# getzlab/rnaseqc

Measured on AMD Instinct MI355X. Metric: reads/sec whole-node (100 M-read synthetic BAM, GENCODE GTF) at 1/2/4/8 GPU -- `value`: the hot path over the records resident in HBM (the bench contract's definition of value); `whole_node.value`: the same job from the BAM file to the reports (CLI `Average Reads/Sec` window), checked against `value, higher is better.
Workload: dtype i32/u64 counters, f64 exon fractions

## Files before the change

rnaseqc_amd/csrc/rsqc_device.h:

```cpp
#pragma once

#if !defined(RSQC_WAVE_EMU)
#include <hip/hip_runtime.h>
#endif
#include <stdint.h>

#include "rsqc_read.h"

#define RSQC_K1_THREADS 256
#define RSQC_MAX_BIAS_WINDOW 1024
#define RSQC_K3_THREADS 1024
#include "rsqc_k3_plan.h"

namespace rsqc {

struct DevBatch {
    uint64_t n;
    uint64_t record_base;
    const rsqc_rec_core *core;
    const rsqc_rec_aux *aux;
    const uint32_t *cigar;
    const uint32_t *qhash2;
    uint32_t n_seg;
    const int32_t *seg_tid;
    const uint64_t *seg_start;
    const uint64_t *seg_file_index;
    uint32_t n_wide;
    const uint64_t *wide_index;
    const int32_t *wide_nm, *wide_l_qseq;
    const uint32_t *wide_n_cigar;
};

RSQC_HD uint64_t batch_file_index(const DevBatch &b, uint32_t seg, uint64_t i) {
    return b.seg_file_index ? b.seg_file_index[seg] + (i - b.seg_start[seg]) : b.record_base + i;
}

struct FragCandidates {
    uint64_t *file_index;
    uint64_t *qhash;
    int32_t *name;
    int32_t *endpos;
    uint32_t *flag_size;
    uint32_t *count; uint32_t cap;
    uint32_t *chunk_count;
    uint32_t *h2;
};

struct DevReference {
    const unsigned long long *bits;
    const unsigned long long *word_off;
    const unsigned long long *length;
};
struct GcCandidates {
    uint64_t *file_index;
    uint64_t *qhash;
    uint32_t *row;
    int32_t *endpos;
    uint32_t *flag_lq;
    int32_t *tid;
    uint32_t *count; uint32_t cap;
    uint32_t *h2;
};
__device__ __forceinline__ uint32_t gc_count(const DevReference &R, int contig, int64_t s, int64_t e) {
    if (e <= s) return 0u;
    const unsigned long long *w = R.bits + R.word_off[contig];
    const int64_t w0 = s >> 6, w1 = (e - 1) >> 6;
    uint32_t n = 0;
    for (int64_t i = w0; i <= w1; ++i) {
        unsigned long long x = w[i];
        if (i == w0) x &= ~0ull << (s & 63);
        if (i == w1) x &= ~0ull >> (63 - ((e - 1) & 63));
        n += (uint32_t)__popcll(x);
    }
    return n;
}
__device__ __forceinline__ double gc_value(uint32_t k, uint64_t size) {
    const double inc = 1.0 / (double)size;
    double c = 0.0;
    for (uint32_t i = 0; i < k; ++i) c += inc;
    return c;
}

struct alignas(16) PairRec { uint32_t gene, h2; uint64_t hash; };
struct DevAccum {
    unsigned long long *gene_reads, *gene_unique, *gene_frag, *counters;
    double *exon_acc;
    uint32_t *cov_diff;
    PairRec *pairs;
    uint32_t pair_chunk_cap; uint32_t *pair_chunk_count;
    uint32_t pair_slow_base, pair_slow_cap; uint32_t *pair_slow_count;
    uint32_t *ovf_count; uint64_t *ovf_index; uint32_t ovf_cap;
    uint32_t *defer_index; uint32_t *defer_list; uint32_t *defer_total;
    uint32_t *tile_span;
    FragCandidates frag;
    uint32_t *rl_stats;
    uint32_t *rl_seg;
    int32_t *read_length;
    int *error;
};

struct GeneCovArgs {
    const uint32_t *ge_off, *ge_row;
    const ExonRow *ex;
    const uint32_t *ex_cov;
    const uint32_t *ex_id;
    const uint32_t *gene_cov_off;
    const uint32_t *gene_coding;
    const uint8_t *gene_flags;
    const uint8_t *gene_owned;
    const uint32_t *gene_order;
    const unsigned long long *gene_reads;
    uint32_t *cov;
    int32_t n_listed;
    uint32_t mask; int32_t bias_offset, bias_window; uint64_t bias_gene_length;
    double *g_mean, *g_std, *g_cv; uint8_t *g_valid;
    double *e_cv; uint8_t *e_cv_valid;
    unsigned long long *bias3, *bias5;
    int *error;
};
void launch_gene_coverage(hipStream_t s, hipStream_t s2, hipStream_t s3, const GeneCovArgs &A, uint32_t n_large, uint32_t n_medium, uint32_t n_xlarge,
                          uint32_t n_le6144 = 0, uint32_t n_le3072 = 0, uint32_t n_le2048 = 0, uint32_t n_le1024 = 0);

void launch_reduce_add(hipStream_t s, unsigned long long *du, const unsigned long long *su, size_t nu, double *df, const double *sf, size_t nf,
                       uint8_t *db, const uint8_t *sb, size_t nb);
void launch_pack_results(hipStream_t s, const double *exon_acc, uint8_t *exon_hit, uint32_t n_exons);
void launch_reset(hipStream_t s, void *arena, size_t arena_bytes, void *cov, size_t cov_bytes, uint32_t *rl_min);
void launch_classify(hipStream_t s, int grid, int variant, const DevAnnotation &a, const DevParams &p, const DevBatch &b,
                     const DevAccum &acc);
inline int rsqc_long_grid(int k1_grid) { return k1_grid < 1024 ? k1_grid : 1024; }
void launch_classify_long(hipStream_t s, int k1_grid, const DevAnnotation &a, const DevParams &p, const DevBatch &b, const DevAccum &acc);
void launch_ei_rank(hipStream_t s, const EiEntry *ei, uint32_t ei_lo, uint32_t ei_hi, EiRank *rank, uint32_t n_words);
void launch_classify_slow(hipStream_t s, const DevAnnotation &a, const DevParams &p, const DevBatch &b,
                          const DevAccum &acc);
#define RSQC_RL_SUMMARY_WORDS (2 + 2 * 128)
void launch_read_length(hipStream_t s, const DevAnnotation &a, const DevParams &p, const DevBatch &b,
                        const DevAccum &acc, uint32_t *summary);
#define RSQC_SLOW_RES 2048u
#define RSQC_SLOW_LEGACY_GRID 4096u
#ifndef RSQC_K4_PART_READS
#define RSQC_K4_PART_READS 1024
#endif
#define RSQC_K4_SUB_CAP (2 * RSQC_K4_PART_READS)
#define RSQC_K4_PART_SLOTS (4 * RSQC_K4_PART_READS)
#ifndef RSQC_K4_COUNT_THREADS
#define RSQC_K4_COUNT_THREADS 256
#endif
struct FragKey { uint32_t lo, hi, h2; };
struct FragPlan {
    uint32_t *part_first;
    uint32_t *cursor;
    uint4 *ginfo;
    uint4 *part_info;
    uint32_t *full_list, *full_n;
    FragKey *list;
    unsigned long long *blk_space; uint32_t *blk_parts;
};
void launch_frag_layout(hipStream_t s, const unsigned long long *gene_reads, uint32_t n_genes, const FragPlan &P, int *error);
void launch_frag_local(hipStream_t s, const DevAccum &acc, uint32_t n_chunks, const FragPlan &P, uint32_t list_blocks);
void launch_pairs_append(hipStream_t s, const PairRec *src, uint32_t chunk_cap, const uint32_t *counts,
                         uint32_t n_chunks, uint32_t slow_base, uint32_t slow_cap, PairRec *dst);
void launch_frag_count(hipStream_t s, uint32_t n_genes, const FragPlan &P, uint32_t parts_bound, unsigned long long *gene_frag, int *error);

}

#include <vector>
namespace rsqc {
struct SortScratch { void *k0 = nullptr, *k1 = nullptr, *v0 = nullptr, *v1 = nullptr, *v2 = nullptr, *v3 = nullptr, *tmp = nullptr, *count = nullptr;
                     size_t cap_n = 0, tmp_bytes = 0; uint32_t *table = nullptr, *out_size = nullptr, *out_count = nullptr; };
void free_sort_scratch(SortScratch &s);
int run_fragment_sizes(hipStream_t stream, const FragCandidates &c, uint32_t n, uint32_t max_samples,
                       std::vector<int64_t> &sizes, std::vector<uint64_t> &counts, uint32_t &remaining, SortScratch &S, uint32_t &n_kept, int *d_error);
void launch_frag_compact(hipStream_t s, const FragCandidates &src, const FragCandidates &dst, uint64_t n_rec, int k1_grid);
void launch_gc_pack(hipStream_t s, const uint8_t *ascii, uint64_t len, unsigned long long *words);
void launch_exon_gc(hipStream_t s, const DevAnnotation &a, const DevReference &R, double *exon_gc);
void launch_gc_candidates(hipStream_t s, const DevAnnotation &a, const DevParams &p, const DevBatch &b, const DevReference &R,
                          const GcCandidates &out, int *error);
int run_gc_content(hipStream_t stream, const GcCandidates &c, uint32_t n, const DevReference &R, unsigned long long *bins, SortScratch &scratch, int *d_error);
}
```

rnaseqc_amd/csrc/rsqc_k4.h:

```cpp
#pragma once

namespace rsqc {


__device__ __forceinline__ uint32_t frag_part_hash(uint64_t key) {
    uint32_t h = (uint32_t)(key >> 32);
    h ^= h >> 15; h *= 0x2C1B3C6Du; h ^= h >> 12;
    return h;
}
__device__ __forceinline__ uint32_t frag_parts_of(unsigned long long reads) {
    return (uint32_t)((reads + RSQC_K4_PART_READS - 1) / RSQC_K4_PART_READS);
}
__device__ __forceinline__ uint32_t frag_cap_of(unsigned long long reads) {
    return frag_parts_of(reads) == 1 ? (uint32_t)reads : (uint32_t)RSQC_K4_SUB_CAP;
}
__device__ __forceinline__ unsigned long long frag_space_of(unsigned long long reads) {
    return ((unsigned long long)frag_parts_of(reads) * frag_cap_of(reads) + 15ull) & ~15ull;
}
__global__ void __launch_bounds__(1024)
frag_layout_totals_kernel(const unsigned long long *gene_reads, uint32_t n_genes, unsigned long long *blk_space, uint32_t *blk_parts, int *error) {
    __shared__ unsigned long long w_space[16];
    __shared__ uint32_t w_parts[16];
    const uint32_t g = blockIdx.x * 1024u + threadIdx.x;
    unsigned long long space = 0; uint32_t parts = 0;
// ... 65 lines not shown
constexpr int k4l_log2(unsigned v) { return v <= 1 ? 0 : 1 + k4l_log2(v >> 1); }
#ifndef RSQC_K4L_WIN
#define RSQC_K4L_WIN 2048
#endif
#ifndef RSQC_K4L_CHUNKS
#define RSQC_K4L_CHUNKS 2
#endif
inline uint32_t frag_local_chunk_wgs(uint32_t n_chunks) { return (n_chunks + RSQC_K4L_CHUNKS - 1u) / RSQC_K4L_CHUNKS; }
struct K4LocalShared {
    uint32_t gkey[RSQC_K4L_GSLOTS], gcnt[RSQC_K4L_GSLOTS];
    unsigned long long win[RSQC_K4L_WIN];
    uint32_t win2[RSQC_K4L_WIN];
};

#ifdef __HIPCC__
#ifndef RSQC_K4L_WAVES
#define RSQC_K4L_WAVES 6
#endif
#define RSQC_K4L_OCC __attribute__((amdgpu_waves_per_eu(RSQC_K4L_WAVES, RSQC_K4L_WAVES)))
#else
#define RSQC_K4L_OCC
#endif
__global__ void __launch_bounds__(RSQC_K4L_THREADS) RSQC_K4L_OCC
frag_local_kernel(const PairRec *pairs, uint32_t chunk_cap,
                  const uint32_t *chunk_count, uint32_t n_chunks, uint32_t slow_base, uint32_t slow_cap,
                  const uint4 *ginfo, uint32_t *cursor, FragKey *list, int *error) {
    __shared__ K4LocalShared S;
    constexpr int CH = RSQC_K4L_CHUNKS;
    const uint32_t n_cwg = (n_chunks + (uint32_t)CH - 1u) / (uint32_t)CH;
    uint32_t cbase[CH], cend[CH];
    uint32_t count, piece0 = 0; constexpr uint32_t piece_step = 1;
    if (blockIdx.x < n_cwg) {
        uint32_t run = 0;
#pragma unroll
        for (int k = 0; k < CH; ++k) {
            const uint32_t c = blockIdx.x * (uint32_t)CH + (uint32_t)k;
            const uint32_t n = c < n_chunks ? (chunk_count[c] < chunk_cap ? chunk_count[c] : chunk_cap) : 0u;
            cbase[k] = c * chunk_cap; run += n; cend[k] = run;
        }
        count = run;
    } else {
#pragma unroll
        for (int k = 0; k < CH; ++k) { cbase[k] = slow_base; cend[k] = 0u; }
        count = chunk_count[n_chunks] < slow_cap ? chunk_count[n_chunks] : slow_cap;
        cend[CH - 1] = count;
#pragma unroll
        for (int k = 0; k < CH - 1; ++k) cend[k] = 0u;
    }
    if (count == 0u) return;
    constexpr int U = RSQC_K4L_PIECE / RSQC_K4L_THREADS;
    constexpr uint32_t NONE = 0xFFFFFFFFu;
    uint32_t n_pieces = (count + RSQC_K4L_PIECE - 1) / RSQC_K4L_PIECE;
    if (blockIdx.x >= n_cwg) {
        const uint32_t sharers = gridDim.x - n_cwg, me = blockIdx.x - n_cwg;
        const uint32_t per = (n_pieces + sharers - 1) / sharers;
        piece0 = me * per < n_pieces ? me * per : n_pieces;
        n_pieces = piece0 + per < n_pieces ? piece0 + per : n_pieces;
    }
    auto pair_at = [&](uint32_t j) -> uint32_t {
        uint32_t at = cbase[CH - 1] + (j - (CH > 1 ? cend[CH - 2] : 0u));
#pragma unroll
        for (int k = CH - 2; k >= 0; --k) if (j < cend[k]) at = cbase[k] + (j - (k > 0 ? cend[k - 1] : 0u));
        return at;
    };
    auto load_piece = [&](uint32_t piece, uint32_t (&g)[U], uint64_t (&key)[U], uint32_t (&h2)[U]) {
#pragma unroll
        for (int u = 0; u < U; ++u) {
            const uint32_t j = piece * RSQC_K4L_PIECE + (uint32_t)u * RSQC_K4L_THREADS + threadIdx.x;
            const bool ok = piece < n_pieces && j < count;
            PairRec r{NONE, 0u, 0ull};
            if (ok) r = pairs[pair_at(j)];
            g[u] = r.gene; key[u] = r.hash; h2[u] = r.h2;
        }
    };
#ifdef RSQC_K1_PROF
    if (blockIdx.x == 1000 && n_chunks > 1000) {
        for (uint32_t i = threadIdx.x; i < count && i < 32768u; i += blockDim.x) { g_dbg_pair_hash[i] = pairs[pair_at(i)].hash; g_dbg_pair_gene[i] = pairs[pair_at(i)].gene; }
        if (threadIdx.x == 0) g_dbg_pair_count = count;
    }
#endif
    uint32_t g[U]; uint64_t key[U]; uint32_t h2[U];
    load_piece(piece0, g, key, h2);
    for (int i = threadIdx.x; i < RSQC_K4L_WIN; i += blockDim.x) { S.win[i] = 0ull; S.win2[i] = 0u; }
    RSQC_FIN_BEGIN
    for (uint32_t piece = piece0; piece < n_pieces; piece += piece_step) {
        RSQC_FIN_SECT(32, 0);
        uint4 gi[U];
#pragma unroll
        for (int u = 0; u < U; ++u) { const uint32_t gq = g[u] != NONE ? g[u] : 0u; gi[u] = ginfo[gq]; }
        uint32_t gn[U]; uint64_t keyn[U]; uint32_t h2n[U];
        load_piece(piece + piece_step, gn, keyn, h2n);
        __syncthreads();
        for (int i = threadIdx.x; i < RSQC_K4L_GSLOTS; i += blockDim.x) { S.gkey[i] = NONE; S.gcnt[i] = 0u; }
        __syncthreads();
        RSQC_FIN_SECT(32, 1);
        uint32_t gp[U], gslot[U], rank[U];
#pragma unroll
        for (int u = 0; u < U; ++u) {
            gslot[u] = NONE; rank[u] = 0; gp[u] = 0;
            if (key[u] == 0) key[u] = 0x9e3779b97f4a7c15ull;
            if (g[u] == NONE) continue;
            {
                unsigned long long lk = key[u] ^ (((unsigned long long)g[u] << 32) | (unsigned long long)(g[u] * 0x9E3779B1u));
                if (lk == 0ull) lk = 1ull;
                static_assert((RSQC_K4L_WIN & (RSQC_K4L_WIN - 1)) == 0, "window size");
                const uint32_t ws = ((((uint32_t)lk ^ (uint32_t)(lk >> 32)) * 0x9E3779B1u) >> 12) & (RSQC_K4L_WIN - 1);
                const bool seen1 = atomicExch(&S.win[ws], lk) == lk, seen2 = atomicExch(&S.win2[ws], h2[u]) == h2[u];
                if (seen1 && seen2) { g[u] = NONE; continue; }
            }
            gp[u] = gi[u].x + (gi[u].y > 1 ? (uint32_t)(((unsigned long long)frag_part_hash(key[u]) * gi[u].y) >> 32) : 0u);
            static_assert((RSQC_K4L_GSLOTS & (RSQC_K4L_GSLOTS - 1)) == 0, "slot hash");
            uint32_t sl = (gp[u] * 0x9E3779B1u) >> (32 - k4l_log2(RSQC_K4L_GSLOTS));
#pragma unroll 1
            for (int probe = 0; probe < 16; ++probe) {
                const uint32_t o = atomicCAS(&S.gkey[sl], NONE, gp[u]);
                if (o == NONE || o == gp[u]) { gslot[u] = sl; rank[u] = atomicAdd(&S.gcnt[sl], 1u); break; }
                sl = (sl + 1) & (RSQC_K4L_GSLOTS - 1);
            }
        }
        RSQC_FIN_SECT(32, 3);
        __syncthreads();
        RSQC_FIN_SECT(32, 4);
        {
            constexpr int R = RSQC_K4L_GSLOTS / RSQC_K4L_THREADS;
            uint32_t pk[R], pc[R], pr[R];
#pragma unroll
            for (int j = 0; j < R; ++j) { pk[j] = S.gkey[j * RSQC_K4L_THREADS + threadIdx.x]; pc[j] = S.gcnt[j * RSQC_K4L_THREADS + threadIdx.x]; }
#pragma unroll
            for (int j = 0; j < R; ++j) pr[j] = pk[j] != NONE ? atomicAdd(&cursor[pk[j]], pc[j]) : 0u;
#pragma unroll
            for (int j = 0; j < R; ++j) S.gcnt[j * RSQC_K4L_THREADS + threadIdx.x] = pr[j];
        }
        __syncthreads();
        RSQC_FIN_SECT(32, 5);
#pragma unroll
        for (int u = 0; u < U; ++u) {
            if (g[u] == NONE) continue;
            const uint32_t at = gslot[u] != NONE ? S.gcnt[gslot[u]] + rank[u] : atomicAdd(&cursor[gp[u]], 1u);
            const uint32_t cap = gi[u].z;
            if (at < cap) {
                const unsigned long long where = ((unsigned long long)gi[u].w << 4) + (unsigned long long)(gp[u] - gi[u].x) * cap + at;
                list[where] = FragKey{(uint32_t)key[u], (uint32_t)(key[u] >> 32), h2[u]};
            } else atomicExch(error, RSQC_ERR_CAPACITY);
        }
        RSQC_FIN_SECT(32, 6);
#ifdef RSQC_K1_PROF
        if (threadIdx.x == 0) atomicAdd(&g_fin_prof[32 + 15], 1ull);
#endif
#pragma unroll
        for (int u = 0; u < U; ++u) { g[u] = gn[u]; key[u] = keyn[u]; h2[u] = h2n[u]; }
    }
}

template <int SLOTS>
__global__ void __launch_bounds__(RSQC_K4_COUNT_THREADS)
frag_count_kernel(const uint32_t *n_parts_at, const uint32_t *cursor, const uint4 *part_info, const FragKey *list,
                  unsigned long long *gene_frag, uint32_t *full_list, uint32_t *full_n, int *error) {
    constexpr bool LISTED = SLOTS == RSQC_K4_PART_SLOTS;
    __shared__ unsigned long long s_keys[SLOTS];
    __shared__ uint32_t s_h2[SLOTS];
    constexpr uint32_t OVF = 32;
    __shared__ unsigned long long s_ovk[OVF];
    __shared__ uint32_t s_ov2[OVF], s_ovn;
    __shared__ uint32_t s_fresh[2];
    constexpr int KPT = (SLOTS / 2) / RSQC_K4_COUNT_THREADS;
    constexpr uint32_t N_LO = SLOTS == RSQC_K4_PART_SLOTS ? (uint32_t)SLOTS / 4u : 0u;
    const uint32_t n_parts = LISTED ? *full_n : *n_parts_at;
    struct Row { uint32_t fill; uint4 info; bool fuller; };
    auto row_of = [&](uint32_t i) -> Row {
        Row r; r.fill = 0u; r.info = make_uint4(0u, 0u, 0u, 0u); r.fuller = false;
        if (i < n_parts) {
            const uint32_t w = LISTED ? full_list[i] : i;
            r.fill = cursor[w]; r.info = part_info[w];
            const uint32_t n = r.fill < r.info.y ? r.fill : r.info.y;
            r.fuller = n > (uint32_t)SLOTS / 2u;
            if (n <= N_LO || r.fuller) r.fill = 0u;
        }
        return r;
    };
    auto keys_of = [&](const Row &r, unsigned long long (&kv)[KPT], uint32_t (&k2)[KPT]) {
        const uint32_t n = r.fill < r.info.y ? r.fill : r.info.y;
        const unsigned long long off = (unsigned long long)r.info.z | ((unsigned long long)r.info.w << 32);
        const FragKey *keys = list + off;
#pragma unroll
        for (int j = 0; j < KPT; ++j) {
            const uint32_t i = (uint32_t)j * RSQC_K4_COUNT_THREADS + threadIdx.x;
            FragKey e{0u, 0u, 0u};
            if (i < n) e = keys[i];
            kv[j] = (unsigned long long)e.lo | ((unsigned long long)e.hi << 32); k2[j] = e.h2;
        }
    };
    uint32_t w = blockIdx.x;
    Row cur = row_of(w), nxt = row_of(w + gridDim.x);
    unsigned long long kv[KPT], kvn[KPT]; uint32_t k2[KPT], k2n[KPT];
    keys_of(cur, kv, k2);
    if (threadIdx.x < 2) s_fresh[threadIdx.x] = 0u;
    if (threadIdx.x == 0) s_ovn = 0u;
    uint32_t round = 0;
    bool owe = false; uint32_t owe_gene = 0u;
    auto settle = [&]() {
        const uint32_t cell = (round - 1u) & 1u;
        uint32_t t = s_fresh[cell]; s_fresh[cell] = 0u;
        if (s_ovn) {
            const uint32_t m = s_ovn < OVF ? s_ovn : OVF;
            for (uint32_t a = 0; a < m; ++a) {
                bool first = true;
                for (uint32_t b2 = 0; b2 < a; ++b2) if (s_ovk[b2] == s_ovk[a] && s_ov2[b2] == s_ov2[a]) first = false;
                if (first) ++t;
            }
            s_ovn = 0u;
        }
        if (t) atomicAdd(&gene_frag[owe_gene], (unsigned long long)t);
    };
#if defined(__HIP_DEVICE_COMPILE__)
#define K4_UNI(x) ((uint32_t)__builtin_amdgcn_readfirstlane((int)(x)))
#else
#define K4_UNI(x) ((uint32_t)(x))
#endif
    RSQC_FIN_BEGIN
    while (w < n_parts) {
        RSQC_FIN_SECT(48, 0);
        const Row nn = row_of(w + 2u * gridDim.x);
        keys_of(nxt, kvn, k2n);
        if (!LISTED && cur.fuller && threadIdx.x == 0) full_list[atomicAdd(full_n, 1u)] = w;
        if (cur.fill != 0u) {
            const uint32_t gene = K4_UNI(cur.info.x), cap = K4_UNI(cur.info.y), fill = K4_UNI(cur.fill);
            const uint32_t n = fill < cap ? fill : cap;
            uint32_t slots = 64;
            while (slots < 2 * n && slots < (uint32_t)SLOTS) slots <<= 1;
            const uint32_t smask = slots - 1;
            for (uint32_t i = threadIdx.x; i < slots; i += blockDim.x) s_keys[i] = 0ull;
            __syncthreads();
            if (owe && threadIdx.x == 0) settle();
            RSQC_FIN_SECT(48, 1);
            uint32_t fresh = 0;
            constexpr uint32_t NO_SLOT = 0xFFFFFFFFu;
            auto insert = [&](unsigned long long k, uint32_t h2) -> uint32_t {
                uint32_t slot = (((uint32_t)k * 0x9E3779B1u) >> 16) & smask;
#pragma unroll 1
                for (uint32_t probe = 0; probe < slots; ++probe) {
                    const unsigned long long old = atomicCAS(&s_keys[slot], 0ull, k);
                    if (old == 0ull) { s_h2[slot] = h2; ++fresh; return NO_SLOT; }
                    if (old == k) return slot;
                    slot = (slot + 1) & smask;
                }
                atomicExch(error, RSQC_ERR_CAPACITY);
                return NO_SLOT;
            };
            uint32_t same[KPT];
#pragma unroll
            for (int j = 0; j < KPT; ++j) same[j] = ((uint32_t)j * RSQC_K4_COUNT_THREADS + threadIdx.x < n) ? insert(kv[j], k2[j]) : NO_SLOT;
            static_assert(RSQC_K4_SUB_CAP <= RSQC_K4_PART_SLOTS / 2 && RSQC_K4_PART_READS <= RSQC_K4_PART_SLOTS / 2, "a list fits the registers of its instance");
            if (n > (uint32_t)KPT * RSQC_K4_COUNT_THREADS) atomicExch(error, RSQC_ERR_CAPACITY);
            __syncthreads();
#pragma unroll
            for (int j = 0; j < KPT; ++j)
                if (same[j] != NO_SLOT && s_h2[same[j]] != k2[j]) {
                    const uint32_t at = atomicAdd(&s_ovn, 1u);
                    if (at < OVF) { s_ovk[at] = kv[j]; s_ov2[at] = k2[j]; } else atomicExch(error, RSQC_ERR_CAPACITY);
                }
            RSQC_FIN_SECT(48, 2);
            fresh = wave_sum_u32_full(fresh);
            if (lane_id() == 0 && fresh) atomicAdd(&s_fresh[round & 1], fresh);
            owe = true; owe_gene = gene;
            ++round;
            RSQC_FIN_SECT(48, 3);
#ifdef RSQC_K1_PROF
            if (threadIdx.x == 0) { atomicAdd(&g_fin_prof[48 + 15], 1ull); atomicAdd(&g_fin_prof[48 + 14], (unsigned long long)n); }
#endif
        }
        w += gridDim.x; cur = nxt; nxt = nn;
#pragma unroll
        for (int j = 0; j < KPT; ++j) { kv[j] = kvn[j]; k2[j] = k2n[j]; }
    }
    if (owe) {
        __syncthreads();
        if (threadIdx.x == 0) settle();
    }
#undef K4_UNI
}

}
```

rnaseqc_amd/csrc/rsqc_kernels.hip:

```cpp
#include <hip/hip_runtime.h>
#include <stdint.h>
#include <algorithm>
#include <cstdlib>

#ifdef RSQC_K1_PROF
namespace rsqc { __device__ __forceinline__ void k1_mark(int sec); __device__ __forceinline__ void k1_event(int id, bool cond); }
#define RSQC_MARK(sec) ::rsqc::k1_mark(sec)
#define RSQC_EVENT(id, cond) ::rsqc::k1_event(id, cond)
#endif

#include "rsqc_device.h"
#ifndef RSQC_K1_PROF
#define RSQC_FIN_STAMP(sec)
#define RSQC_FIN_SECT(base, sec)
#define RSQC_FIN_BEGIN
#endif

namespace rsqc {

}
#include "rsqc_wave.h"
namespace rsqc {

#ifdef RSQC_K1_PROF
// ... 188 lines not shown
    if (w >= n_words) return;
    uint32_t lo = ei_lo, hi = ei_hi;
    while (lo < hi) { const uint32_t m = lo + ((hi - lo) >> 1); if (((uint32_t)ei[m].pos >> 6) < w) lo = m + 1; else hi = m; }
    EiRank r = {0u, 0u, lo, 0u};
    for (uint32_t j = lo; j < ei_hi && ((uint32_t)ei[j].pos >> 6) == w; ++j) {
        const uint32_t bit = (uint32_t)ei[j].pos & 63u;
        if (bit < 32) r.lo |= 1u << bit; else r.hi |= 1u << (bit - 32);
    }
    rank[w] = r;
}
void launch_ei_rank(hipStream_t s, const EiEntry *ei, uint32_t ei_lo, uint32_t ei_hi, EiRank *rank, uint32_t n_words) {
    if (n_words) hipLaunchKernelGGL(ei_rank_kernel, dim3((n_words + 255) / 256), dim3(256), 0, s, ei, ei_lo, ei_hi, rank, n_words);
}

}
#include "rsqc_kr.h"
namespace rsqc {

#define RSQC_K4_SLOW_BLOCKS 32

__global__ void __launch_bounds__(256)
pairs_append_kernel(const PairRec *src, uint32_t chunk_cap, const uint32_t *counts, uint32_t n_chunks,
                    uint32_t slow_base, uint32_t slow_cap, PairRec *dst_pairs) {
    __shared__ unsigned long long s_part[256];
    const uint32_t k = blockIdx.x < n_chunks ? blockIdx.x : n_chunks;
    unsigned long long before = 0;
    for (uint32_t j = threadIdx.x; j < k; j += blockDim.x) before += counts[j] < chunk_cap ? counts[j] : chunk_cap;
    s_part[threadIdx.x] = before;
    __syncthreads();
    for (int o = 128; o > 0; o >>= 1) { if ((int)threadIdx.x < o) s_part[threadIdx.x] += s_part[threadIdx.x + o]; __syncthreads(); }
    const unsigned long long dst = s_part[0];
    uint32_t base, count, lo = 0, step = 1;
    if (blockIdx.x < n_chunks) { base = blockIdx.x * chunk_cap; count = counts[k] < chunk_cap ? counts[k] : chunk_cap; }
    else { base = slow_base; count = counts[n_chunks] < slow_cap ? counts[n_chunks] : slow_cap; lo = blockIdx.x - n_chunks; step = gridDim.x - n_chunks; }
    for (uint32_t i = lo * blockDim.x + threadIdx.x; i < count; i += step * blockDim.x) {
        dst_pairs[dst + i] = src[base + i];
    }
}
void launch_pairs_append(hipStream_t s, const PairRec *src, uint32_t chunk_cap, const uint32_t *counts,
                         uint32_t n_chunks, uint32_t slow_base, uint32_t slow_cap, PairRec *dst) {
    hipLaunchKernelGGL(pairs_append_kernel, dim3(n_chunks + RSQC_K4_SLOW_BLOCKS), dim3(256), 0, s, src, chunk_cap, counts,
                       n_chunks, slow_base, slow_cap, dst);
}

}
#include "rsqc_k4.h"
namespace rsqc {

}
#include "rsqc_k3.h"
namespace rsqc {

}
#include "rsqc_gc.h"
namespace rsqc {

void launch_gc_pack(hipStream_t s, const uint8_t *ascii, uint64_t len, unsigned long long *words) {
    const uint64_t n_words = (len + 63) / 64;
    if (!n_words) return;
    hipLaunchKernelGGL(gc_pack_kernel, dim3((unsigned)std::min<uint64_t>((n_words + 255) / 256, 65536)), dim3(256), 0, s, ascii, len, words);
}
void launch_exon_gc(hipStream_t s, const DevAnnotation &a, const DevReference &R, double *exon_gc) {
    if (a.n_exons <= 0) return;
    hipLaunchKernelGGL(exon_gc_kernel, dim3((a.n_exons + 255) / 256), dim3(256), 0, s, a, R, exon_gc);
}
void launch_gc_candidates(hipStream_t s, const DevAnnotation &a, const DevParams &p, const DevBatch &b, const DevReference &R,
                          const GcCandidates &out, int *error) {
    if (!b.n) return;
    const uint64_t blocks = (b.n + GC_CAND_THREADS - 1) / GC_CAND_THREADS;
    hipLaunchKernelGGL(gc_candidates_kernel, dim3((unsigned)std::min<uint64_t>(blocks, 4096)), dim3(GC_CAND_THREADS), 0, s, a, p, b, R, out, error);
}

__global__ void __launch_bounds__(256)
pack_results_kernel(const double *exon_acc, uint8_t *exon_hit, uint32_t n_exons) {
    for (uint32_t i = blockIdx.x * blockDim.x + threadIdx.x; i < n_exons; i += gridDim.x * blockDim.x) exon_hit[i] = exon_acc[i] > 0.0 ? 1 : 0;
}

__global__ void __launch_bounds__(256)
reset_kernel(uint4 *arena, size_t arena_vec, uint4 *cov, size_t cov_vec, size_t rl_vec) {
    const size_t stride = (size_t)gridDim.x * blockDim.x;
    const uint4 z = {0u, 0u, 0u, 0u}, armed = {0u, 0xFFFFFFFFu, 0u, 0u};
    for (size_t i = (size_t)blockIdx.x * blockDim.x + threadIdx.x; i < cov_vec; i += stride) cov[i] = z;
    for (size_t i = (size_t)blockIdx.x * blockDim.x + threadIdx.x; i < arena_vec; i += stride) arena[i] = i == rl_vec ? armed : z;
}

__global__ void __launch_bounds__(256)
reduce_add_kernel(unsigned long long *du, const unsigned long long *su, size_t nu, double *df, const double *sf, size_t nf,
                  uint8_t *db, const uint8_t *sb, size_t nb) {
    const size_t stride = (size_t)gridDim.x * blockDim.x, t = (size_t)blockIdx.x * blockDim.x + threadIdx.x;
    for (size_t i = t; i < nu; i += stride) du[i] += su[i];
    for (size_t i = t; i < nf; i += stride) df[i] += sf[i];
    for (size_t i = t; i < nb; i += stride) db[i] = (uint8_t)(db[i] + sb[i]);
}
void launch_reduce_add(hipStream_t s, unsigned long long *du, const unsigned long long *su, size_t nu, double *df, const double *sf, size_t nf,
                       uint8_t *db, const uint8_t *sb, size_t nb) {
    hipLaunchKernelGGL(reduce_add_kernel, dim3(512), dim3(256), 0, s, du, su, nu, df, sf, nf, db, sb, nb);
}

void launch_pack_results(hipStream_t s, const double *exon_acc, uint8_t *exon_hit, uint32_t n_exons) {
    if (n_exons) hipLaunchKernelGGL(pack_results_kernel, dim3((n_exons + 255) / 256 < 1024 ? (n_exons + 255) / 256 : 1024), dim3(256), 0, s, exon_acc, exon_hit, n_exons);
}
void launch_reset(hipStream_t s, void *arena, size_t arena_bytes, void *cov, size_t cov_bytes, uint32_t *rl_min) {
    const size_t rl_vec = (size_t)((char *)rl_min - 4 - (char *)arena) / 16;
    hipLaunchKernelGGL(reset_kernel, dim3(1024), dim3(256), 0, s, (uint4 *)arena, (arena_bytes + 15) / 16, (uint4 *)cov, (cov_bytes + 15) / 16, rl_vec);
}
void launch_frag_compact(hipStream_t s, const FragCandidates &src, const FragCandidates &dst, uint64_t n_rec, int k1_grid) {
    hipLaunchKernelGGL(frag_compact_kernel, dim3(k1_grid), dim3(256), 0, s, src, dst, (uint32_t)n_rec, (uint32_t)k1_grid);
}
void launch_classify(hipStream_t s, int grid, int variant, const DevAnnotation &a, const DevParams &p, const DevBatch &b,
                     const DevAccum &acc) {
    if (variant < 0) hipLaunchKernelGGL(classify_count_kernel_legacy, dim3(grid), dim3(RSQC_K1_THREADS), 0, s, a, p, b, acc);
    else {
#if defined(RSQC_K1_PROF) || defined(RSQC_DIAG_KNOBS)
        static const unsigned pad = getenv("RSQC_K1_LDS_PAD") ? (unsigned)atoi(getenv("RSQC_K1_LDS_PAD")) : 0u;
#else
        const unsigned pad = 0u;
#endif
        const K1Args A{a, p, b, acc};
        if (a.have_bed) hipLaunchKernelGGL(classify_ei_kernel<true>, dim3(grid), dim3(RSQC_K1_THREADS), pad, s, A);
        else hipLaunchKernelGGL(classify_ei_kernel<false>, dim3(grid), dim3(RSQC_K1_THREADS), pad, s, A);
    }
}
void launch_classify_long(hipStream_t s, int k1_grid, const DevAnnotation &a, const DevParams &p, const DevBatch &b, const DevAccum &acc) {
    const K1Args A{a, p, b, acc};
    hipLaunchKernelGGL(classify_long_kernel, dim3((unsigned)rsqc_long_grid(k1_grid)), dim3(RSQC_K1_THREADS), 0, s, A, (uint32_t)k1_grid);
}
void launch_classify_slow(hipStream_t s, const DevAnnotation &a, const DevParams &p, const DevBatch &b,
                          const DevAccum &acc) {
    if (p.legacy) {
        const uint64_t blocks = (b.n + RSQC_SLOW_THREADS - 1) / RSQC_SLOW_THREADS;
        hipLaunchKernelGGL(classify_slow_kernel<true>, dim3((unsigned)std::min<uint64_t>(blocks ? blocks : 1, RSQC_SLOW_LEGACY_GRID)), dim3(RSQC_SLOW_THREADS), 0, s, a, p, b, acc);
    } else {
        const uint64_t blocks = std::max<uint64_t>(64, std::min<uint64_t>(2048, b.n / 200 / RSQC_SLOW_THREADS + 1));
        hipLaunchKernelGGL(classify_slow_kernel<false>, dim3((unsigned)blocks), dim3(RSQC_SLOW_THREADS), 0, s, a, p, b, acc);
    }
}
void launch_read_length(hipStream_t s, const DevAnnotation &a, const DevParams &p, const DevBatch &b,
                        const DevAccum &acc, uint32_t *summary) {
    hipLaunchKernelGGL(read_length_kernel, dim3(acc.rl_seg ? b.n_seg : 1u), dim3(64), 0, s, a, p, b, acc, summary);
}
void launch_frag_layout(hipStream_t s, const unsigned long long *gene_reads, uint32_t n_genes, const FragPlan &P, int *error) {
    const uint32_t blocks = (n_genes + 1023u) / 1024u;
    if (!blocks) return;
    hipLaunchKernelGGL(frag_layout_totals_kernel, dim3(blocks), dim3(1024), 0, s, gene_reads, n_genes, P.blk_space, P.blk_parts, error);
    hipLaunchKernelGGL(frag_layout_kernel, dim3(blocks), dim3(1024), 0, s, gene_reads, n_genes, P.blk_space, P.blk_parts, P.part_first,
                       P.ginfo, P.cursor, P.part_info, P.full_n);
}
void launch_frag_local(hipStream_t s, const DevAccum &acc, uint32_t n_chunks, const FragPlan &P, uint32_t list_blocks) {
    hipLaunchKernelGGL(frag_local_kernel, dim3(frag_local_chunk_wgs(n_chunks) + (list_blocks ? list_blocks : RSQC_K4_SLOW_BLOCKS)), dim3(RSQC_K4L_THREADS), 0, s, acc.pairs, acc.pair_chunk_cap, acc.pair_chunk_count, n_chunks, acc.pair_slow_base, acc.pair_slow_cap,
                       P.ginfo, P.cursor, P.list, acc.error);
}
void launch_frag_count(hipStream_t s, uint32_t n_genes, const FragPlan &P, uint32_t parts_bound, unsigned long long *gene_frag, int *error) {
    if (n_genes == 0) return;
    const uint32_t grid = parts_bound < 16384u ? (parts_bound ? parts_bound : 1u) : 16384u;
    hipLaunchKernelGGL((frag_count_kernel<RSQC_K4_PART_SLOTS / 2>), dim3(grid), dim3(RSQC_K4_COUNT_THREADS), 0, s, P.part_first + n_genes, P.cursor, P.part_info, P.list, gene_frag,
                       P.full_list, P.full_n, error);
    hipLaunchKernelGGL((frag_count_kernel<RSQC_K4_PART_SLOTS>), dim3(grid < 1024u ? grid : 1024u), dim3(RSQC_K4_COUNT_THREADS), 0, s, P.part_first + n_genes, P.cursor, P.part_info, P.list, gene_frag,
                       P.full_list, P.full_n, error);
}
#ifndef RSQC_K3_MEDIUM_T
#define RSQC_K3_MEDIUM_T uint32_t
#endif
#ifndef RSQC_K3_SMALL_T
#define RSQC_K3_SMALL_T uint32_t
#endif
void launch_gene_coverage(hipStream_t s, hipStream_t s2, hipStream_t s3, const GeneCovArgs &A, uint32_t n_large, uint32_t n_medium, uint32_t n_xlarge,
                          uint32_t n_le6144, uint32_t n_le3072, uint32_t n_le2048, uint32_t n_le1024) {
    if (A.n_listed <= 0) return;
    K3Launch plan[RSQC_K3_LAUNCHES];
    k3_plan((uint32_t)A.n_listed, n_large, n_medium, n_xlarge, n_le6144, n_le3072, n_le2048, n_le1024, plan);
    const hipStream_t streams[3] = {s, s2, s3};
    const bool wide = A.bias_window > 128;
#define RSQC_K3_LAUNCH(K, T, COVT, CAP)                                                                                  \
    case K: {                                                                                                            \
        static_assert(T == K3_THREADS[K] && CAP == K3_CAPS[K], "the instance of a launch is the one its plan entry describes"); \
        if (wide) hipLaunchKernelGGL((gene_coverage_kernel<T, RSQC_MAX_BIAS_WINDOW, COVT, CAP>), dim3(L.count), dim3(T), 0, streams[L.stream], A, L.first); \
        else hipLaunchKernelGGL((gene_coverage_kernel<T, 128, COVT, CAP>), dim3(L.count), dim3(T), 0, streams[L.stream], A, L.first);  \
    } break;
    for (int k = 0; k < RSQC_K3_LAUNCHES; ++k) {
        const K3Launch &L = plan[k];
        if (!L.count) continue;
        switch (k) {
            RSQC_K3_LAUNCH(0, 1024, uint16_t, RSQC_K3_LARGE_LDS16)
            RSQC_K3_LAUNCH(1, 256, RSQC_K3_MEDIUM_T, RSQC_K3_MEDIUM_MAX)
            RSQC_K3_LAUNCH(2, 256, RSQC_K3_MEDIUM_T, 6144)
            RSQC_K3_LAUNCH(3, 1024, uint16_t, RSQC_K3_LARGE2_LDS16)
            RSQC_K3_LAUNCH(4, 64, RSQC_K3_SMALL_T, RSQC_K3_SMALL_MAX)
            RSQC_K3_LAUNCH(5, 64, RSQC_K3_SMALL_T, 3072)
            RSQC_K3_LAUNCH(6, 64, RSQC_K3_SMALL_T, 2048)
            RSQC_K3_LAUNCH(7, 64, RSQC_K3_SMALL_T, 1024)
        }
    }
#undef RSQC_K3_LAUNCH
}

}
```

Baseline: 26.66 billion.

## Handle small fragment partitions per wave in frag_count kernel

Restructures the fragment-count kernel so each block loads 64 partitions at once. Small partitions (up to an eighth of the slots) are deduplicated by a single wavefront in its own quarter of the LDS hash set, using only wave-level barriers. Wider partitions, and small ones whose secondary hash disagrees, fall back to the block-wide path. This is meant to cut per-partition block barriers and idle threads on tiny partitions, at the cost of more complex control flow and an extra block barrier per batch.

```diff
diff --git a/rnaseqc_amd/csrc/rsqc_device.h b/rnaseqc_amd/csrc/rsqc_device.h
--- a/rnaseqc_amd/csrc/rsqc_device.h
+++ b/rnaseqc_amd/csrc/rsqc_device.h
@@ -145,6 +145,9 @@
 #ifndef RSQC_K4_COUNT_THREADS
 #define RSQC_K4_COUNT_THREADS 256
 #endif
+#ifndef RSQC_K4_COUNT_GRID
+#define RSQC_K4_COUNT_GRID 16384u
+#endif
 struct FragKey { uint32_t lo, hi, h2; };
 struct FragPlan {
     uint32_t *part_first;
diff --git a/rnaseqc_amd/csrc/rsqc_k4.h b/rnaseqc_amd/csrc/rsqc_k4.h
--- a/rnaseqc_amd/csrc/rsqc_k4.h
+++ b/rnaseqc_amd/csrc/rsqc_k4.h
@@ -241,6 +241,26 @@
     }
 }
 
+__device__ __forceinline__ void k4_wave_lds_visible() {
+    __builtin_amdgcn_fence(__ATOMIC_RELEASE, "wavefront");
+    __builtin_amdgcn_wave_barrier();
+    __builtin_amdgcn_fence(__ATOMIC_ACQUIRE, "wavefront");
+}
+constexpr uint32_t K4_NO_SLOT = 0xFFFFFFFFu;
+__device__ __forceinline__ uint32_t frag_set_insert(unsigned long long *set, uint32_t *set_h2, uint32_t slots, unsigned long long k, uint32_t h2,
+                                                    uint32_t &fresh, int *error) {
+    const uint32_t smask = slots - 1u;
+    uint32_t slot = (((uint32_t)k * 0x9E3779B1u) >> 16) & smask;
+#pragma unroll 1
+    for (uint32_t probe = 0; probe < slots; ++probe) {
+        const unsigned long long old = atomicCAS(&set[slot], 0ull, k);
+        if (old == 0ull) { set_h2[slot] = h2; ++fresh; return K4_NO_SLOT; }
+        if (old == k) return slot;
+        slot = (slot + 1u) & smask;
+    }
+    atomicExch(error, RSQC_ERR_CAPACITY);
+    return K4_NO_SLOT;
+}
 template <int SLOTS>
 __global__ void __launch_bounds__(RSQC_K4_COUNT_THREADS)
 frag_count_kernel(const uint32_t *n_parts_at, const uint32_t *cursor, const uint4 *part_info, const FragKey *list,
@@ -255,22 +275,35 @@
     constexpr int KPT = (SLOTS / 2) / RSQC_K4_COUNT_THREADS;
     constexpr uint32_t N_LO = SLOTS == RSQC_K4_PART_SLOTS ? (uint32_t)SLOTS / 4u : 0u;
     const uint32_t n_parts = LISTED ? *full_n : *n_parts_at;
-    struct Row { uint32_t fill; uint4 info; bool fuller; };
-    auto row_of = [&](uint32_t i) -> Row {
-        Row r; r.fill = 0u; r.info = make_uint4(0u, 0u, 0u, 0u); r.fuller = false;
+    static_assert(RSQC_K4_COUNT_THREADS == 256, "four waves: the small path gives each a quarter of the set");
+    constexpr int WAVES = RSQC_K4_COUNT_THREADS / 64;
+    constexpr uint32_t W_SMALL = LISTED ? 0u : (uint32_t)SLOTS / 8u;
+    constexpr uint32_t QSLOTS = (uint32_t)SLOTS / WAVES;
+    constexpr int SKPT = LISTED ? 1 : (int)(W_SMALL / 64u);
+    static_assert(LISTED || 2u * W_SMALL <= QSLOTS, "a small partition fits its wave's quarter at half load");
+    __shared__ uint32_t s_defer[2][2];
+    const int l = lane_id(), wv = (int)(threadIdx.x >> 6);
+    struct Rows { uint32_t n, gene, off_lo, off_hi; };
+    auto rows_at = [&](unsigned long long base) -> Rows {
+        Rows r{0u, 0u, 0u, 0u};
+        const unsigned long long i = base + (unsigned long long)l * gridDim.x;
         if (i < n_parts) {
-            const uint32_t w = LISTED ? full_list[i] : i;
-            r.fill = cursor[w]; r.info = part_info[w];
-            const uint32_t n = r.fill < r.info.y ? r.fill : r.info.y;
-            r.fuller = n > (uint32_t)SLOTS / 2u;
-            if (n <= N_LO || r.fuller) r.fill = 0u;
+            const uint32_t w = LISTED ? full_list[i] : (uint32_t)i;
+            const uint32_t fill = cursor[w]; const uint4 info = part_info[w];
+            r.n = fill < info.y ? fill : info.y; r.gene = info.x; r.off_lo = info.z; r.off_hi = info.w;
         }
         return r;
     };
-    auto keys_of = [&](const Row &r, unsigned long long (&kv)[KPT], uint32_t (&k2)[KPT]) {
-        const uint32_t n = r.fill < r.info.y ? r.fill : r.info.y;
-        const unsigned long long off = (unsigned long long)r.info.z | ((unsigned long long)r.info.w << 32);
-        const FragKey *keys = list + off;
+    const unsigned long long step = 64ull * gridDim.x;
+    unsigned long long base = blockIdx.x;
+    Rows R = rows_at(base);
+    auto list_of = [&](int src) -> const FragKey * {
+        return list + ((unsigned long long)lane_value(R.off_lo, src) | ((unsigned long long)lane_value(R.off_hi, src) << 32));
+    };
+    auto keys_of = [&](int at, unsigned long long (&kv)[KPT], uint32_t (&k2)[KPT]) {
+        const int src = at < 0 ? 0 : at;
+        const uint32_t n = at < 0 ? 0u : lane_value(R.n, src);
+        const FragKey *keys = list_of(src);
 #pragma unroll
         for (int j = 0; j < KPT; ++j) {
             const uint32_t i = (uint32_t)j * RSQC_K4_COUNT_THREADS + threadIdx.x;
@@ -279,13 +312,11 @@
             kv[j] = (unsigned long long)e.lo | ((unsigned long long)e.hi << 32); k2[j] = e.h2;
         }
     };
-    uint32_t w = blockIdx.x;
-    Row cur = row_of(w), nxt = row_of(w + gridDim.x);
-    unsigned long long kv[KPT], kvn[KPT]; uint32_t k2[KPT], k2n[KPT];
-    keys_of(cur, kv, k2);
     if (threadIdx.x < 2) s_fresh[threadIdx.x] = 0u;
     if (threadIdx.x == 0) s_ovn = 0u;
-    uint32_t round = 0;
+    if (threadIdx.x < 4) s_defer[threadIdx.x >> 1][threadIdx.x & 1] = 0u;
+    __syncthreads();
+    uint32_t round = 0, batch = 0;
     bool owe = false; uint32_t owe_gene = 0u;
     auto settle = [&]() {
         const uint32_t cell = (round - 1u) & 1u;
@@ -307,44 +338,98 @@
 #define K4_UNI(x) ((uint32_t)(x))
 #endif
     RSQC_FIN_BEGIN
-    while (w < n_parts) {
+    while (base < n_parts) {
         RSQC_FIN_SECT(48, 0);
-        const Row nn = row_of(w + 2u * gridDim.x);
-        keys_of(nxt, kvn, k2n);
-        if (!LISTED && cur.fuller && threadIdx.x == 0) full_list[atomicAdd(full_n, 1u)] = w;
-        if (cur.fill != 0u) {
-            const uint32_t gene = K4_UNI(cur.info.x), cap = K4_UNI(cur.info.y), fill = K4_UNI(cur.fill);
-            const uint32_t n = fill < cap ? fill : cap;
+        const Rows RN = rows_at(base + step);
+        const bool is_small = R.n != 0u && R.n <= W_SMALL;
+        const bool is_wide = R.n > (LISTED ? N_LO : W_SMALL) && R.n <= (uint32_t)SLOTS / 2u;
+        unsigned long long wide = __ballot(is_wide);
+        if constexpr (!LISTED) {
+            if (wv == 0 && R.n > (uint32_t)SLOTS / 2u) full_list[atomicAdd(full_n, 1u)] = (uint32_t)(base + (unsigned long long)l * gridDim.x);
+        }
+        if constexpr (!LISTED) {
+            const unsigned long long small = __ballot(is_small);
+            unsigned long long todo = __ballot(is_small && (mask_rank(small) & (uint32_t)(WAVES - 1)) == (uint32_t)wv);
+            unsigned long long *q_keys = s_keys + (uint32_t)wv * QSLOTS; uint32_t *q_h2 = s_h2 + (uint32_t)wv * QSLOTS;
+            auto small_keys_of = [&](int at, unsigned long long (&a)[SKPT], uint32_t (&a2)[SKPT]) {
+                const int src = at < 0 ? 0 : at;
+                const uint32_t n = at < 0 ? 0u : lane_value(R.n, src);
+                const FragKey *keys = list_of(src);
+#pragma unroll
+                for (int j = 0; j < SKPT; ++j) {
+                    const uint32_t i = (uint32_t)(j * 64 + l);
+                    FragKey e{0u, 0u, 0u};
+                    if (i < n) e = keys[i];
+                    a[j] = (unsigned long long)e.lo | ((unsigned long long)e.hi << 32); a2[j] = e.h2;
+                }
+            };
+            unsigned long long sk[SKPT], skn[SKPT]; uint32_t s2[SKPT], s2n[SKPT];
+            int sc = -1;
+            if (todo) { sc = __ffsll(todo) - 1; todo &= todo - 1ull; }
+            small_keys_of(sc, sk, s2);
+            while (sc >= 0) {
+                int sn = -1;
+                if (todo) { sn = __ffsll(todo) - 1; todo &= todo - 1ull; }
+                small_keys_of(sn, skn, s2n);
+                const uint32_t n = lane_value(R.n, sc), gene = lane_value(R.gene, sc);
+                uint32_t slots = 64;
+                while (slots < 2u * n) slots <<= 1;
+                for (uint32_t i = (uint32_t)l; i < slots; i += 64u) q_keys[i] = 0ull;
+                k4_wave_lds_visible();
+                uint32_t fresh = 0, same[SKPT];
+#pragma unroll
+                for (int j = 0; j < SKPT; ++j) same[j] = ((uint32_t)(j * 64 + l) < n) ? frag_set_insert(q_keys, q_h2, slots, sk[j], s2[j], fresh, error) : K4_NO_SLOT;
+                k4_wave_lds_visible();
+                bool differs = false;
+#pragma unroll
+                for (int j = 0; j < SKPT; ++j) if (same[j] != K4_NO_SLOT && q_h2[same[j]] != s2[j]) differs = true;
+                if (__ballot(differs)) {
+                    if (l == 0) atomicAdd(&s_defer[batch & 1u][sc >> 5], 1u << (sc & 31));
+                } else {
+                    fresh = wave_sum_u32_full(fresh);
+                    if (l == 0 && fresh) atomicAdd(&gene_frag[gene], (unsigned long long)fresh);
+                }
+#ifdef RSQC_K1_PROF
+                if (l == 0) { atomicAdd(&g_fin_prof[48 + 5], 1ull); atomicAdd(&g_fin_prof[48 + 6], (unsigned long long)n); }
+#endif
+                sc = sn;
+#pragma unroll
+                for (int j = 0; j < SKPT; ++j) { sk[j] = skn[j]; s2[j] = s2n[j]; }
+            }
+        }
+        __syncthreads();
+        RSQC_FIN_SECT(48, 4);
+        unsigned long long handed = 0ull;
+        if constexpr (!LISTED) {
+            handed = (unsigned long long)K4_UNI(s_defer[batch & 1u][0]) | ((unsigned long long)K4_UNI(s_defer[batch & 1u][1]) << 32);
+            if (threadIdx.x < 2) s_defer[(batch + 1u) & 1u][threadIdx.x] = 0u;
+        }
+        unsigned long long kv[KPT], kvn[KPT]; uint32_t k2[KPT], k2n[KPT];
+        int cur = -1;
+        if (wide) { cur = __ffsll(wide) - 1; wide &= wide - 1ull; }
+        else if (handed) { cur = __ffsll(handed) - 1; handed &= handed - 1ull; }
+        keys_of(cur, kv, k2);
+        while (cur >= 0) {
+            int nx = -1;
+            if (wide) { nx = __ffsll(wide) - 1; wide &= wide - 1ull; }
+            else if (handed) { nx = __ffsll(handed) - 1; handed &= handed - 1ull; }
+            keys_of(nx, kvn, k2n);
+            const uint32_t gene = lane_value(R.gene, cur), n = lane_value(R.n, cur);
             uint32_t slots = 64;
             while (slots < 2 * n && slots < (uint32_t)SLOTS) slots <<= 1;
-            const uint32_t smask = slots - 1;
             for (uint32_t i = threadIdx.x; i < slots; i += blockDim.x) s_keys[i] = 0ull;
             __syncthreads();
             if (owe && threadIdx.x == 0) settle();
             RSQC_FIN_SECT(48, 1);
-            uint32_t fresh = 0;
-            constexpr uint32_t NO_SLOT = 0xFFFFFFFFu;
-            auto insert = [&](unsigned long long k, uint32_t h2) -> uint32_t {
-                uint32_t slot = (((uint32_t)k * 0x9E3779B1u) >> 16) & smask;
-#pragma unroll 1
-                for (uint32_t probe = 0; probe < slots; ++probe) {
-                    const unsigned long long old = atomicCAS(&s_keys[slot], 0ull, k);
-                    if (old == 0ull) { s_h2[slot] = h2; ++fresh; return NO_SLOT; }
-                    if (old == k) return slot;
-                    slot = (slot + 1) & smask;
-                }
-                atomicExch(error, RSQC_ERR_CAPACITY);
-                return NO_SLOT;
-            };
-            uint32_t same[KPT];
-#pragma unroll
-            for (int j = 0; j < KPT; ++j) same[j] = ((uint32_t)j * RSQC_K4_COUNT_THREADS + threadIdx.x < n) ? insert(kv[j], k2[j]) : NO_SLOT;
+            uint32_t fresh = 0, same[KPT];
+#pragma unroll
+            for (int j = 0; j < KPT; ++j) same[j] = ((uint32_t)j * RSQC_K4_COUNT_THREADS + threadIdx.x < n) ? frag_set_insert(s_keys, s_h2, slots, kv[j], k2[j], fresh, error) : K4_NO_SLOT;
             static_assert(RSQC_K4_SUB_CAP <= RSQC_K4_PART_SLOTS / 2 && RSQC_K4_PART_READS <= RSQC_K4_PART_SLOTS / 2, "a list fits the registers of its instance");
             if (n > (uint32_t)KPT * RSQC_K4_COUNT_THREADS) atomicExch(error, RSQC_ERR_CAPACITY);
             __syncthreads();
 #pragma unroll
             for (int j = 0; j < KPT; ++j)
-                if (same[j] != NO_SLOT && s_h2[same[j]] != k2[j]) {
+                if (same[j] != K4_NO_SLOT && s_h2[same[j]] != k2[j]) {
                     const uint32_t at = atomicAdd(&s_ovn, 1u);
                     if (at < OVF) { s_ovk[at] = kv[j]; s_ov2[at] = k2[j]; } else atomicExch(error, RSQC_ERR_CAPACITY);
                 }
@@ -357,14 +442,20 @@
 #ifdef RSQC_K1_PROF
             if (threadIdx.x == 0) { atomicAdd(&g_fin_prof[48 + 15], 1ull); atomicAdd(&g_fin_prof[48 + 14], (unsigned long long)n); }
 #endif
-        }
-        w += gridDim.x; cur = nxt; nxt = nn;
-#pragma unroll
-        for (int j = 0; j < KPT; ++j) { kv[j] = kvn[j]; k2[j] = k2n[j]; }
-    }
-    if (owe) {
-        __syncthreads();
-        if (threadIdx.x == 0) settle();
+            cur = nx;
+#pragma unroll
+            for (int j = 0; j < KPT; ++j) { kv[j] = kvn[j]; k2[j] = k2n[j]; }
+        }
+        __syncthreads();
+        if (owe) {
+            if (threadIdx.x == 0) settle();
+            owe = false;
+        }
+        RSQC_FIN_SECT(48, 7);
+#ifdef RSQC_K1_PROF
+        if (threadIdx.x == 0) atomicAdd(&g_fin_prof[48 + 8], 1ull);
+#endif
+        base += step; R = RN; ++batch;
     }
 #undef K4_UNI
 }
diff --git a/rnaseqc_amd/csrc/rsqc_kernels.hip b/rnaseqc_amd/csrc/rsqc_kernels.hip
--- a/rnaseqc_amd/csrc/rsqc_kernels.hip
+++ b/rnaseqc_amd/csrc/rsqc_kernels.hip
@@ -364,7 +364,7 @@
 }
 void launch_frag_count(hipStream_t s, uint32_t n_genes, const FragPlan &P, uint32_t parts_bound, unsigned long long *gene_frag, int *error) {
     if (n_genes == 0) return;
-    const uint32_t grid = parts_bound < 16384u ? (parts_bound ? parts_bound : 1u) : 16384u;
+    const uint32_t grid = parts_bound < RSQC_K4_COUNT_GRID ? (parts_bound ? parts_bound : 1u) : RSQC_K4_COUNT_GRID;
     hipLaunchKernelGGL((frag_count_kernel<RSQC_K4_PART_SLOTS / 2>), dim3(grid), dim3(RSQC_K4_COUNT_THREADS), 0, s, P.part_first + n_genes, P.cursor, P.part_info, P.list, gene_frag,
                        P.full_list, P.full_n, error);
     hipLaunchKernelGGL((frag_count_kernel<RSQC_K4_PART_SLOTS>), dim3(grid < 1024u ? grid : 1024u), dim3(RSQC_K4_COUNT_THREADS), 0, s, P.part_first + n_genes, P.cursor, P.part_info, P.list, gene_frag,
```

New measurement: 26.95 billion (median of 6 runs). No clear change (+1.1%).
